# OrangeEarth15/3dgrut

Measured on AMD Instinct MI355X. Metric: train-step images/sec + render ms/frame, MipNeRF360 bicycle @1/2/4/8 GPU, higher is better.
Workload: dtype f32; 1 GPU; bicycle_like_6M_1237x822; num_gaussians=6000000, sh_degree=3, parallelism=per-view dp1, exchanged_records_last_step=0, loss=0.8*L1+0.2*(1-SSIM) (HIP fused SSIM), optimizer=HIP fused SH-gradient+Adam, all 59 params/Gaussian, trainer=native, optimizer_state=synthetic mid-training state: non-zero Adam moments on every row, storage_order=morton, optimizer_overlap=True, lazy_moment_decay=True, densification_statistics=False, warmup_extended_by=6

## Files before the change

3dgrut_amd/_capi.py:

```python
import ctypes as C
import os

HERE = os.path.dirname(os.path.abspath(__file__))
LIB_PATH = os.environ.get("GUT_HIP_LIB", os.path.join(HERE, "libgut_hip.so"))

GUT_ABI_VERSION = 6
GUT_NUM_KERNEL_TIMERS = 11
BWD_RAW_PARAMETER_GRADS = 1
BWD_COMPACT_RADIANCE_GRADS = 2
BWD_SKIP_EPILOGUE = 4
OPT_LAZY_TILE_ORDER = 1
ADAM_CLEAR_CONSUMED_GRADS = 1
GRADIENT_RECORD_FLOATS = 16
OPT_SORTED_REFERENCE_BACKWARD = 2
OPT_EARLY_EXTRA_PERCENT = 3
OPT_FORWARD_TILE_ORDER = 4
OPT_KERNEL_TIMING_SET = 5
OPT_DEBUG_REPLACE_SCRATCH = 100
KERNEL_TIMER_NAMES = ("project", "scan", "expand", "sort", "ranges", "render", "render_bwd", "project_bwd", "optimizer",
                      "optimizer_early", "optimizer_early_2")

SHUTTER_GLOBAL = 4
CAMERA_PINHOLE, CAMERA_FISHEYE = 0, 1

BUF = dict(tiles_count=0, tiles_offset=1, proj_pos=2, conic_opacity=3, extent=4, depth=5, feat=6,
           unsorted_keys=7, unsorted_ids=8, sorted_keys=9, sorted_ids=10, tile_ranges=11, grad_scratch=12,
           tile_traversed_fwd=13, tile_traversed_bwd=14, ordered_ids=15, packed_rows=16)


class GutCamera(C.Structure):
    _fields_ = [
        ("model", C.c_int32), ("shutter", C.c_int32),
        ("principal_point", C.c_float * 2), ("focal_length", C.c_float * 2),
        ("radial_coeffs", C.c_float * 6), ("tangential_coeffs", C.c_float * 2), ("thin_prism_coeffs", C.c_float * 4),
        ("max_angle", C.c_float), ("pose_start", C.c_float * 7), ("pose_end", C.c_float * 7),
        ("timestamp_start_us", C.c_int64), ("timestamp_end_us", C.c_int64),
    ]


class GutConfig(C.Structure):
    _fields_ = [
        ("abi_version", C.c_int32), ("enable_kernel_timings", C.c_int32), ("particle_radiance_sph_degree", C.c_int32),
        ("particle_kernel_degree", C.c_int32), ("k_buffer_size", C.c_int32), ("global_z_order", C.c_int32),
        ("n_rolling_shutter_iterations", C.c_int32), ("ut_require_all_sigma_points", C.c_int32),
        ("rect_bounding", C.c_int32), ("tight_opacity_bounding", C.c_int32), ("tile_based_culling", C.c_int32),
        ("enable_hitcounts", C.c_int32),
        ("particle_kernel_min_response", C.c_float), ("particle_kernel_min_alpha", C.c_float),
        ("particle_kernel_max_alpha", C.c_float), ("min_transmittance", C.c_float),
        ("ut_alpha", C.c_float), ("ut_beta", C.c_float), ("ut_kappa", C.c_float), ("ut_in_image_margin_factor", C.c_float),
    ]


class GutStats(C.Structure):
    _fields_ = [
        ("num_particles", C.c_uint64), ("num_visible", C.c_uint64), ("num_intersections", C.c_uint64),
        ("num_tiles", C.c_uint64), ("num_pixels", C.c_uint64), ("traversed_fwd", C.c_uint64),
        ("traversed_bwd", C.c_uint64), ("sort_end_bit", C.c_uint32), ("binning_overflows", C.c_uint32),
        ("side_stream_rows", C.c_uint64), ("side_stream_rows_first_launch", C.c_uint64),
    ]


class GutLazyMoments(C.Structure):
    _fields_ = [("d_wave_step", C.c_void_p), ("d_pow_beta1", C.c_void_p), ("d_pow_beta2", C.c_void_p), ("table_len", C.c_uint32),
                ("d_overrun", C.c_void_p)]


class GutRegularisation(C.Structure):
    _fields_ = [("density_coeff", C.c_float), ("scale_coeff", C.c_float), ("d_partials", C.c_void_p)]


EXPORTS = ("gut_default_config", "gut_create", "gut_destroy", "gut_trace", "gut_trace_bwd", "gut_collect_times",
           "gut_get_stats", "gut_debug_buffer", "gut_debug_copy", "gut_kernel_times", "gut_kernel_times_mean", "gut_last_error", "gut_abi_version",
           "gut_ssim_workspace_bytes", "gut_ssim_forward", "gut_ssim_backward",
           "gut_photometric_workspace_bytes", "gut_photometric_loss", "gut_optimize_after_bwd", "gut_set_option",
           "gut_trace_bwd_ex", "gut_optimize_rows_without_gradient", "gut_compact_gradient_rows", "gut_scatter_gradient_records",
           "gut_sh_adam_step_ex", "gut_mark_walked_waves", "gut_adam_unwalked_waves", "gut_activate_pack", "gut_adam_step", "gut_sh_adam_step", "gut_mcmc_relocation",
           "gut_optimize_finish_without_gradient", "gut_scatter_gradient_records_dev", "gut_adam_unwalked_waves_ex", "gut_sync_moments", "gut_trace_fields", "gut_trace_bwd_fields", "gut_selective_adam",
           "gut_trace_model_fields", "gut_trace_bwd_model_fields", "gut_position_gradient_statistics",
           "gut_set_position_gradient_statistics", "gut_mcmc_perturb", "gut_trace_raw_model_fields", "gut_set_regularisation",
           "gut_sh_adam_step_regularised", "gut_adam_unwalked_waves_regularised", "gut_sync_moments_ex", "gut_regularisation_gradient",
# ... 97 lines not shown
```

3dgrut_amd/csrc/gut_api.cpp:

```cpp
#include <hip/hip_runtime.h>

#include <cmath>
#include <cstdarg>
#include <cstdio>
#include <cstdlib>
#include <cstring>
#include <deque>
#include <mutex>
#include <new>
#include <string>

#include "gut_internal.h"

namespace {

thread_local std::string g_last_error;

int fail(const char* fmt, ...) {
    char buf[512];
    va_list ap;
    va_start(ap, fmt);
    vsnprintf(buf, sizeof(buf), fmt, ap);
    va_end(ap);
    g_last_error = buf;
// ... 1332 lines not shown
    case GUT_BUF_UNSORTED_KEYS:
    case GUT_BUF_UNSORTED_IDS:
    case GUT_BUF_SORTED_KEYS:
    case GUT_BUF_SORTED_IDS:
        if (h->lazy_order && !h->dbg_unsorted_valid && m) {
            DeviceGuard dev_guard;
            HIP_TRY(dev_guard.set(h->device));
            HIP_TRY(h->keys_unsorted.ensure(8 * m));
            HIP_TRY(h->ids_unsorted.ensure(4 * m));
            gut::launch_expand(h->fwd_stream, h->view, h->consts, (uint32_t)n, h->tiles_count.as<uint32_t>(), h->wave_sums.as<uint32_t>(),
                               h->block_prefix.as<uint32_t>(), h->scan_total.as<uint32_t>(), h->proj_pos.as<float>(),
                               h->conic_opacity.as<float>(), h->extent.as<float>(), h->depth.as<float>(),
                               h->keys_unsorted.as<uint64_t>(), h->ids_unsorted.as<uint32_t>(), (uint32_t)m);
            HIP_TRY(hipStreamSynchronize(h->fwd_stream));
            h->dbg_unsorted_valid = true;
        }
        if (which == GUT_BUF_UNSORTED_KEYS) { *d_ptr = h->keys_unsorted.p; *bytes = 8 * m; break; }
        if (which == GUT_BUF_UNSORTED_IDS) { *d_ptr = h->ids_unsorted.p; *bytes = 4 * m; break; }
        if (h->lazy_order) {
            if (!h->dbg_sorted_valid && m) {
                DeviceGuard dev_guard;
                HIP_TRY(dev_guard.set(h->device));
                HIP_TRY(h->dbg_keys_sorted.ensure(8 * m));
                HIP_TRY(h->dbg_ids_sorted.ensure(4 * m));
                DevBuf tmp;
                HIP_TRY(tmp.ensure(gut::sort_temp_bytes((uint32_t)m, h->end_bit)));
                hipError_t e = gut::run_sort(h->fwd_stream, tmp.p, tmp.cap, h->keys_unsorted.as<uint64_t>(),
                                             h->dbg_keys_sorted.as<uint64_t>(), h->ids_unsorted.as<uint32_t>(),
                                             h->dbg_ids_sorted.as<uint32_t>(), (uint32_t)m, h->end_bit);
                if (e == hipSuccess) e = hipStreamSynchronize(h->fwd_stream);
                tmp.release();
                HIP_TRY(e);
                h->dbg_sorted_valid = true;
            }
            if (which == GUT_BUF_SORTED_KEYS) { *d_ptr = h->dbg_keys_sorted.p; *bytes = 8 * m; }
            else { *d_ptr = h->dbg_ids_sorted.p; *bytes = 4 * m; }
        } else if (which == GUT_BUF_SORTED_KEYS) { *d_ptr = h->keys_sorted.p; *bytes = 8 * m; }
        else { *d_ptr = h->ids_sorted.p; *bytes = 4 * m; }
        break;
    case GUT_BUF_ORDERED_IDS:
        if (h->lazy_order && !h->dbg_ordered_valid && m) {
            DeviceGuard dev_guard;
            HIP_TRY(dev_guard.set(h->device));
            gut::launch_mask_unordered(h->fwd_stream, (uint32_t)h->tiles, h->ranges.as<uint32_t>(), h->tile_ordered.as<uint32_t>(),
                                       h->ids_ordered.as<uint32_t>());
            HIP_TRY(hipStreamSynchronize(h->fwd_stream));
            h->dbg_ordered_valid = true;
        }
        *d_ptr = h->lazy_order ? h->ids_ordered.p : h->ids_sorted.p; *bytes = 4 * m; break;
    case GUT_BUF_PACKED_ROWS:
        if (!h->packed_valid) return fail("gut_debug_buffer: the last forward was not a field-wise one (no packed rows)");
        *d_ptr = h->packed12.p; *bytes = 48 * n; break;
    case GUT_BUF_TILE_RANGES: *d_ptr = h->ranges.p; *bytes = 8 * t; break;
    case GUT_BUF_GRAD_SCRATCH:
        if (!h->have_backward) return fail("gut_debug_buffer: no backward yet");
        *d_ptr = h->grad16.p; *bytes = 64 * n; break;
    case GUT_BUF_TILE_TRAVERSED_FWD: *d_ptr = h->trav_fwd.p; *bytes = 4 * t; break;
    case GUT_BUF_TILE_TRAVERSED_BWD:
        if (!h->have_backward) return fail("gut_debug_buffer: no backward yet");
        *d_ptr = h->trav_bwd.p; *bytes = 4 * t; break;
    default: return fail("gut_debug_buffer: unknown buffer %d", which);
    }
    return 0;
}

int gut_debug_copy(gut_handle h, int32_t which, void* d_dst, size_t bytes) {
    void* src = nullptr;
    size_t have = 0;
    if (gut_debug_buffer(h, which, &src, &have)) return 1;
    if (bytes < have) return fail("gut_debug_copy: destination holds %zu bytes, buffer has %zu", bytes, have);
    if (have == 0) return 0;
    std::lock_guard<std::mutex> lock(h->mu);
    DeviceGuard dev_guard;
    HIP_TRY(dev_guard.set(h->device));
    HIP_TRY(hipMemcpyAsync(d_dst, src, have, hipMemcpyDeviceToDevice, h->fwd_stream));
    HIP_TRY(hipStreamSynchronize(h->fwd_stream));
    return 0;
}

}
```

3dgrut_amd/csrc/gut_project.hip:

```cpp
#include "gut_internal.h"

namespace gut {

__device__ __forceinline__ uint32_t f2u(float f) { return __float_as_uint(f); }
__device__ __forceinline__ float u2f(uint32_t u) { return __uint_as_float(u); }

__device__ float det_logf(float x) {
    uint32_t ix = f2u(x);
    int k = 0;
    if (ix >= 0x7f800000u) return x;
    if (ix < 0x00800000u) {
        if (ix == 0) return -__builtin_inff();
        x = x * 33554432.0f;
        ix = f2u(x);
        k -= 25;
    }
    k += (int)(ix >> 23) - 127;
    ix &= 0x007fffffu;
    const uint32_t i = (ix + (0x95f64u << 3)) & 0x800000u;
    x = u2f(ix | (i ^ 0x3f800000u));
    k += (int)(i >> 23);
    const float f = x - 1.0f;
    const float s = f / (2.0f + f);
    const float dk = (float)k;
// ... 222 lines not shown
        }
    }
}

__device__ __forceinline__ int clamp_tile(float v, int grid) {
    if (!(v > 0.0f)) return 0;
    if (v >= (float)grid) return grid;
    return (int)v;
}

struct TileBox {
    int x0, y0, x1, y1;
};

__device__ __forceinline__ TileBox tile_bbox(int gx, int gy, float px, float py, float ex, float ey) {
    TileBox b;
    b.x0 = clamp_tile(floorf((px - 0.5f - ex) / 16.0f), gx);
    b.y0 = clamp_tile(floorf((py - 0.5f - ey) / 16.0f), gy);
    b.x1 = clamp_tile(ceilf((px - 0.5f + ex) / 16.0f), gx);
    b.y1 = clamp_tile(ceilf((py - 0.5f + ey) / 16.0f), gy);
    return b;
}

__device__ __forceinline__ float saturate(float v) { return v > 0.0f ? (v < 1.0f ? v : 1.0f) : 0.0f; }

__device__ float tile_min_power(float tx, float ty, float c0, float c1, float c2, float mx, float my) {
    const float ts = 16.0f;
    const float tminx = ts * tx, tminy = ts * ty;
    const float tmaxx = ts + tminx, tmaxy = ts + tminy;
    const float offx = tminx - mx, offy = tminy - my;
    const float lax = offx > 0.0f ? 1.0f : 0.0f, lay = offy > 0.0f ? 1.0f : 0.0f;
    const float nrx = lax + (mx > tmaxx ? 1.0f : 0.0f);
    const float nry = lay + (my > tmaxy ? 1.0f : 0.0f);
    if ((nrx + nry) > 0.0f) {
        const float px = lax > 0.0f ? tminx : tmaxx;
        const float py = lay > 0.0f ? tminy : tmaxy;
        const float dxx = copysignf(ts, offx), dxy = copysignf(ts, offy);
        const float dfx = mx - px, dfy = my - py;
        const float rcx = 1.0f / (ts * ts * c0);
        const float rcy = 1.0f / (ts * ts * c2);
        const float tx_ = nry * saturate((dxx * c0 * dfx + dxx * c1 * dfy) * rcx);
        const float ty_ = nrx * saturate((dxy * c1 * dfx + dxy * c2 * dfy) * rcy);
        const float qx = mx - (px + tx_ * dxx);
        const float qy = my - (py + ty_ * dxy);
        return 0.5f * (c0 * qx * qx + c2 * qy * qy) + c1 * qx * qy;
    }
    return 0.0f;
}

constexpr int kSerialTiles = 12;
constexpr int kShRow = 49;

constexpr int kBinWindow = 1536;

struct TileWindow {
    int x0, y0, w, h;
};

__device__ TileWindow tile_window(const TileBox& bb, bool small, uint32_t* bins, int* red , uint32_t tid) {
    constexpr int kNone = 0x7fffffff;
    int a = small ? bb.x0 : kNone, b = small ? bb.y0 : kNone, c = small ? -bb.x1 : kNone, d = small ? -bb.y1 : kNone;
#pragma unroll
    for (int o = 32; o > 0; o >>= 1) {
        a = min(a, __shfl_xor(a, o));
        b = min(b, __shfl_xor(b, o));
        c = min(c, __shfl_xor(c, o));
        d = min(d, __shfl_xor(d, o));
    }
    if ((tid & 63u) == 0u) {
        red[4 * (tid >> 6) + 0] = a;
        red[4 * (tid >> 6) + 1] = b;
        red[4 * (tid >> 6) + 2] = c;
        red[4 * (tid >> 6) + 3] = d;
    }
    __syncthreads();
    a = __builtin_amdgcn_readfirstlane(min(min(red[0], red[4]), min(red[8], red[12])));
    b = __builtin_amdgcn_readfirstlane(min(min(red[1], red[5]), min(red[9], red[13])));
    c = __builtin_amdgcn_readfirstlane(min(min(red[2], red[6]), min(red[10], red[14])));
    d = __builtin_amdgcn_readfirstlane(min(min(red[3], red[7]), min(red[11], red[15])));
    TileWindow W = {0, 0, 0, 0};
    if (a != kNone && (-c - a) * (-d - b) <= kBinWindow) W = TileWindow{a, b, -c - a, -d - b};
    for (int k = (int)tid; k < W.w * W.h; k += kBlock) bins[k] = 0u;
    __syncthreads();
    return W;
}

__device__ __forceinline__ bool in_window(const TileWindow& W, int x, int y, uint32_t& bin) {
    const uint32_t bx = (uint32_t)(x - W.x0), by = (uint32_t)(y - W.y0);
    bin = by * (uint32_t)W.w + bx;
    return bx < (uint32_t)W.w && by < (uint32_t)W.h;
}

__device__ __forceinline__ uint32_t window_tile(const TileWindow& W, int grid_x, uint32_t bin) {
    const uint32_t by = bin / (uint32_t)W.w;
    return (uint32_t)(W.y0 + (int)by) * (uint32_t)grid_x + (uint32_t)W.x0 + (bin - by * (uint32_t)W.w);
}

__device__ __forceinline__ float bcast(float v, int src_lane) { return __shfl(v, src_lane); }
__device__ __forceinline__ int bcast(int v, int src_lane) { return __shfl(v, src_lane); }

template <int kVariant, bool kRolling, bool kSplitSH>
__global__ __launch_bounds__(kBlock, 5) void k_project_on_tiles(ViewParams v, RenderConsts c, uint32_t n, int sh_degree,
                                                            const float4* __restrict__ density12,
                                                            const float* __restrict__ sph48,
                                                            const float* __restrict__ sph_albedo,
                                                            uint32_t* __restrict__ tiles_count, float2* __restrict__ proj_pos,
                                                            float4* __restrict__ conic_opacity, float2* __restrict__ extent,
                                                            float* __restrict__ depth, float* __restrict__ feat,
                                                            float* __restrict__ visibility, uint32_t* __restrict__ wave_sums,
                                                            FrameClears clr) {
    __shared__ float sh_lds[(kBlock / 64) * 32 * kShRow];
    __shared__ uint32_t s_bins[kBinWindow];
    __shared__ int s_red[16];
    const uint32_t i = blockIdx.x * kBlock + threadIdx.x;
    const int lane = (int)(threadIdx.x & 63);
    const int wave = (int)(threadIdx.x >> 6);
    for (uint32_t t = i; t < clr.tiles; t += gridDim.x * kBlock) {
        clr.ranges[t] = make_uint2(0u, 0u);
        clr.trav_bwd[t] = 0u;
    }
    if (lane == 0 && clr.wave_walked) clr.wave_walked[blockIdx.x * (kBlock / 64) + (uint32_t)wave] = 0;
    if (i == 0 && clr.cam_pos) {
        clr.cam_pos[0] = v.s2w.t[0]; clr.cam_pos[1] = v.s2w.t[1]; clr.cam_pos[2] = v.s2w.t[2];
    }
    uint32_t cnt = 0;
    bool conic_ok = false, ok = false;
    float cx = 0.f, cy = 0.f, con0 = 0.f, con1 = 0.f, con2 = 0.f, con3 = 0.f, ex = 0.f, ey = 0.f, zkey = 0.f;
    float f0 = 0.f, f1 = 0.f, f2 = 0.f, max_power = 0.f, zcam = 0.f;
    float4 a = make_float4(0.f, 0.f, 0.f, 0.f);
    const uint32_t wave_first = blockIdx.x * kBlock + (uint32_t)wave * 64u;
    const uint32_t rows_here = wave_first < n ? min(64u, n - wave_first) : 0u;
    if (i < n) {
        a = density12[3 * (size_t)i + 0];
        const float4 b = density12[3 * (size_t)i + 1];
// ... 406 lines not shown
    if (serial) {
        for (int y = bb.y0; (y < bb.y1) && (off < max_off); ++y)
            for (int x = bb.x0; (x < bb.x1) && (off < max_off); ++x)
                if (tile_min_power((float)x, (float)y, con.x, con.y, con.z, p.x, p.y) < max_power) {
                    keys[off] = ((uint64_t)(uint32_t)(y * v.grid_x + x) << 32) | dkey;
                    ids[off] = i;
                    off++;
                }
    }
    unsigned long long todo = __ballot(active && area > kSerialTiles);
    while (todo) {
        const int j = __ffsll((long long)todo) - 1;
        todo &= todo - 1;
        const int jx0 = bcast(bb.x0, j), jy0 = bcast(bb.y0, j), jw = bcast(bb.x1 - bb.x0, j), jarea = bcast(area, j);
        const float j0 = bcast(con.x, j), j1 = bcast(con.y, j), j2 = bcast(con.z, j), jcx = bcast(p.x, j), jcy = bcast(p.y, j),
                    jmp = bcast(max_power, j);
        const uint32_t jdkey = (uint32_t)bcast((int)dkey, j), jmax = (uint32_t)bcast((int)max_off, j);
        const uint32_t jid = blockIdx.x * kBlock + (threadIdx.x & ~63u) + (uint32_t)j;
        uint32_t joff = (uint32_t)bcast((int)off, j);
        for (int base = 0; base < jarea; base += 64) {
            const int t = base + lane;
            bool pass = false;
            int tx = 0, ty = 0;
            if (t < jarea) {
                ty = t / jw;
                tx = t - ty * jw;
                pass = tile_min_power((float)(jx0 + tx), (float)(jy0 + ty), j0, j1, j2, jcx, jcy) < jmp;
            }
            const unsigned long long mask = __ballot(pass);
            const uint32_t my = joff + (uint32_t)__popcll(mask & ((1ull << lane) - 1ull));
            if (pass && my < jmax) {
                keys[my] = ((uint64_t)(uint32_t)((jy0 + ty) * v.grid_x + (jx0 + tx)) << 32) | jdkey;
                ids[my] = jid;
            }
            joff += (uint32_t)__popcll(mask);
        }
        if (lane == j) off = joff < jmax ? joff : jmax;
    }
    if (active)
        for (; off < max_off; ++off) {
            keys[off] = ((uint64_t)kInvalid << 32) | f2u(3.4028235e+38f);
            ids[off] = kInvalid;
        }
}

__global__ __launch_bounds__(kBlock) void k_expand_grouped(ViewParams v, RenderConsts c, uint32_t n,
                                                          const float2* __restrict__ proj_pos,
                                                          const float4* __restrict__ conic_opacity,
                                                          const float2* __restrict__ extent, const float* __restrict__ depth,
                                                          uint32_t tiles, const uint32_t* __restrict__ tile_start,
                                                          uint32_t* __restrict__ tile_cursor, uint2* __restrict__ ranges,
                                                          uint2* __restrict__ entries, uint32_t capacity) {
    __shared__ uint32_t s_bins[kBinWindow];
    __shared__ int s_red[16];
    const uint32_t i = blockIdx.x * kBlock + threadIdx.x;
    const int lane = (int)(threadIdx.x & 63);
    for (uint32_t t = i; t < tiles; t += gridDim.x * kBlock) {
        const uint32_t b = tile_start[t], e = tile_start[t + 1];
        ranges[t] = b == e ? make_uint2(0u, 0u) : make_uint2(min(b, capacity), min(e, capacity));
    }
    bool active = false;
    float2 e = make_float2(0.f, 0.f), p = make_float2(0.f, 0.f);
    float4 con = make_float4(0.f, 0.f, 0.f, 0.f);
    uint32_t dkey = 0;
    float max_power = 0.f;
    TileBox bb = {0, 0, 0, 0};
    int area = 0;
    if (i < n) {
        e = extent[i];
        active = !(e.x <= 1e-06f);
    }
    if (active) {
        dkey = f2u(depth[i]);
        p = proj_pos[i];
        bb = tile_bbox(v.grid_x, v.grid_y, p.x, p.y, e.x, e.y);
        area = (bb.x1 - bb.x0) * (bb.y1 - bb.y0);
        con = conic_opacity[i];
        if (c.tile_culling) max_power = det_logf(con.w / c.alpha_threshold);
    }
    const TileWindow W = tile_window(bb, active && area > 0 && area <= kSerialTiles, s_bins, s_red, threadIdx.x);
    auto enumerate = [&](auto emit) {
        if (!c.tile_culling) {
            if (active)
                for (int y = bb.y0; y < bb.y1; ++y)
                    for (int x = bb.x0; x < bb.x1; ++x) emit(x, y, i, dkey);
            return;
        }
        if (active && area <= kSerialTiles)
            for (int y = bb.y0; y < bb.y1; ++y)
                for (int x = bb.x0; x < bb.x1; ++x)
                    if (tile_min_power((float)x, (float)y, con.x, con.y, con.z, p.x, p.y) < max_power) emit(x, y, i, dkey);
        unsigned long long todo = __ballot(active && area > kSerialTiles);
        while (todo) {
            const int j = __ffsll((long long)todo) - 1;
            todo &= todo - 1;
            const int jx0 = bcast(bb.x0, j), jy0 = bcast(bb.y0, j), jw = bcast(bb.x1 - bb.x0, j), jarea = bcast(area, j);
            const float j0 = bcast(con.x, j), j1 = bcast(con.y, j), j2 = bcast(con.z, j), jcx = bcast(p.x, j), jcy = bcast(p.y, j),
                        jmp = bcast(max_power, j);
            const uint32_t jdkey = (uint32_t)bcast((int)dkey, j);
            const uint32_t jid = blockIdx.x * kBlock + (threadIdx.x & ~63u) + (uint32_t)j;
            for (int base = 0; base < jarea; base += 64) {
                const int t = base + lane;
                if (t < jarea) {
                    const int ty = t / jw;
                    const int tx = t - ty * jw;
                    if (tile_min_power((float)(jx0 + tx), (float)(jy0 + ty), j0, j1, j2, jcx, jcy) < jmp) emit(jx0 + tx, jy0 + ty, jid, jdkey);
                }
            }
        }
    };
    enumerate([&](int x, int y, uint32_t, uint32_t) {
        uint32_t bin;
        if (in_window(W, x, y, bin)) atomicAdd(&s_bins[bin], 1u);
    });
    __syncthreads();
    for (int k = (int)threadIdx.x; k < W.w * W.h; k += kBlock) {
        const uint32_t cnt = s_bins[k];
        if (cnt) s_bins[k] = atomicAdd(&tile_cursor[window_tile(W, v.grid_x, (uint32_t)k)], cnt);
    }
    __syncthreads();
    enumerate([&](int x, int y, uint32_t id, uint32_t dk) {
        uint32_t bin;
        const uint32_t slot = in_window(W, x, y, bin) ? atomicAdd(&s_bins[bin], 1u)
                                                      : atomicAdd(&tile_cursor[(uint32_t)y * (uint32_t)v.grid_x + (uint32_t)x], 1u);
        if (slot < capacity) entries[slot] = make_uint2(dk, id);
    });
}

__global__ __launch_bounds__(kBlock) void k_pad_keys(const uint32_t* __restrict__ count, uint32_t sort_n, uint64_t* __restrict__ keys,
                                                    uint32_t* __restrict__ ids) {
    const uint32_t m = *count;
    for (uint32_t k = m + blockIdx.x * kBlock + threadIdx.x; k < sort_n; k += gridDim.x * kBlock) {
        keys[k] = ((uint64_t)kInvalid << 32) | f2u(3.4028235e+38f);
        ids[k] = kInvalid;
    }
}

__global__ __launch_bounds__(kBlock) void k_mask_unordered(uint32_t tiles, const uint2* __restrict__ ranges,
                                                          const uint32_t* __restrict__ tile_ordered, uint32_t* __restrict__ ordered_ids) {
    const uint32_t t = blockIdx.x;
    if (t >= tiles) return;
    const uint2 r = ranges[t];
    for (uint32_t k = r.x + min(r.y - r.x, tile_ordered[t]) + threadIdx.x; k < r.y; k += kBlock) ordered_ids[k] = kInvalid;
}

void launch_mask_unordered(hipStream_t s, uint32_t tiles, const uint32_t* ranges, const uint32_t* tile_ordered, uint32_t* ordered_ids) {
    if (tiles == 0) return;
    hipLaunchKernelGGL(k_mask_unordered, dim3(tiles), dim3(kBlock), 0, s, tiles, reinterpret_cast<const uint2*>(ranges), tile_ordered,
                       ordered_ids);
}

void launch_pad_keys(hipStream_t s, const uint32_t* count, uint32_t sort_n, uint64_t* keys, uint32_t* ids) {
    if (sort_n == 0) return;
    hipLaunchKernelGGL(k_pad_keys, dim3(64), dim3(kBlock), 0, s, count, sort_n, keys, ids);
}

__global__ __launch_bounds__(kBlock) void k_tile_ranges(uint32_t m, const uint64_t* __restrict__ sorted_keys,
                                                       uint2* __restrict__ ranges) {
    const uint32_t k = blockIdx.x * kBlock + threadIdx.x;
    if (k >= m) return;
    const uint32_t tile = (uint32_t)(sorted_keys[k] >> 32);
    const bool valid = tile != kInvalid;
    if (k == 0) {
        if (valid) ranges[tile].x = 0;
    } else {
        const uint32_t prev = (uint32_t)(sorted_keys[k - 1] >> 32);
        if (prev != tile) {
            if (prev != kInvalid) ranges[prev].y = k;
            if (valid) ranges[tile].x = k;
        }
    }
    if (valid && (k == m - 1)) ranges[tile].y = m;
}

template <bool kRawGrads, bool kSplitSH>
__global__ __launch_bounds__(kBlock) void k_project_backward(ViewParams v, uint32_t n, int sh_degree,
                                                            const float4* __restrict__ density12,
// ... 261 lines not shown
```

3dgrut_amd/tracer.py:

```python
import ctypes as C
import enum
import math
import os

import numpy as np
import torch

from . import _capi
from .cameras import ShutterType as DatasetShutterType
from .pose import SensorPose3D, sensor_pose_from_c2w


class ShutterType(enum.IntEnum):
    ROLLING_TOP_TO_BOTTOM = 0
    ROLLING_LEFT_TO_RIGHT = 1
    ROLLING_BOTTOM_TO_TOP = 2
    ROLLING_RIGHT_TO_LEFT = 3
    GLOBAL = 4


SHUTTER_TYPE_MAP = {d: ShutterType[d.name] for d in DatasetShutterType}


def plugin_shutter_type(value):
# ... 400 lines not shown
        with torch.cuda.device(act12.device):
            rc = self._lib.gut_compact_gradient_rows(self._handle, C.c_void_p(stream), act12.data_ptr(), records.data_ptr(),
                                                     int(records.shape[0]), count.data_ptr())
        _capi.check(rc, "compact_gradient_rows")

    def collect_times(self):
        f, b = C.c_float(-1.0), C.c_float(-1.0)
        _capi.check(self._lib.gut_collect_times(self._handle, C.byref(f), C.byref(b)), "collect_times")
        if f.value >= 0:
            self._timings["forward_render"] = f.value
        if b.value >= 0:
            self._timings["backward_render"] = b.value
        return dict(self._timings)

    def set_lazy_tile_order(self, on=True):
        _capi.check(self._lib.gut_set_option(self._handle, _capi.OPT_LAZY_TILE_ORDER, 1 if on else 0), "set_option")

    def set_early_extra_percent(self, percent):
        _capi.check(self._lib.gut_set_option(self._handle, _capi.OPT_EARLY_EXTRA_PERCENT, int(percent)), "set_option")

    def set_forward_tile_order(self, mode):
        _capi.check(self._lib.gut_set_option(self._handle, _capi.OPT_FORWARD_TILE_ORDER, int(mode)), "set_option")

    def set_kernel_timing_set(self, which):
        _capi.check(self._lib.gut_set_option(self._handle, _capi.OPT_KERNEL_TIMING_SET, int(which)), "set_option")

    def debug_replace_scratch(self, index):
        _capi.check(self._lib.gut_set_option(self._handle, _capi.OPT_DEBUG_REPLACE_SCRATCH, int(index)), "set_option")

    def set_sorted_reference_backward(self, on=True):
        _capi.check(self._lib.gut_set_option(self._handle, _capi.OPT_SORTED_REFERENCE_BACKWARD, 1 if on else 0), "set_option")

    def stats(self):
        s = _capi.GutStats()
        _capi.check(self._lib.gut_get_stats(self._handle, C.byref(s)), "stats")
        return {k: int(getattr(s, k)) for k, _ in s._fields_ if k != "reserved"}

    def kernel_times(self):
        arr = (C.c_float * _capi.GUT_NUM_KERNEL_TIMERS)()
        _capi.check(self._lib.gut_kernel_times(self._handle, arr), "kernel_times")
        return dict(zip(_capi.KERNEL_TIMER_NAMES, [float(v) for v in arr]))

    def kernel_times_mean(self):
        arr = (C.c_float * _capi.GUT_NUM_KERNEL_TIMERS)()
        cnt = C.c_int32(0)
        _capi.check(self._lib.gut_kernel_times_mean(self._handle, arr, C.byref(cnt)), "kernel_times_mean")
        return dict(zip(_capi.KERNEL_TIMER_NAMES, [float(v) for v in arr])), int(cnt.value)

    def debug_buffer(self, name, device=None):
        ptr, nbytes = C.c_void_p(), C.c_size_t()
        _capi.check(self._lib.gut_debug_buffer(self._handle, _capi.BUF[name], C.byref(ptr), C.byref(nbytes)), "debug_buffer")
        dt = {"tiles_count": torch.int32, "tiles_offset": torch.int32, "unsorted_ids": torch.int32,
              "sorted_ids": torch.int32, "ordered_ids": torch.int32, "tile_ranges": torch.int32, "tile_traversed_fwd": torch.int32,
              "tile_traversed_bwd": torch.int32, "unsorted_keys": torch.int64,
              "sorted_keys": torch.int64}.get(name, torch.float32)
        n = nbytes.value // (8 if dt == torch.int64 else 4)
        dev = torch.device("cuda", self.device_index) if device is None else device
        out = torch.empty(n, dtype=dt, device=dev)
        if n:
            _capi.check(self._lib.gut_debug_copy(self._handle, _capi.BUF[name], C.c_void_p(out.data_ptr()),
                                                 C.c_size_t(nbytes.value)), "debug_copy")
        return out


class Tracer:
    class _Autograd(torch.autograd.Function):
        @staticmethod
        def forward(ctx, tracer_wrapper, frame_id, n_active_features, ray_ori, ray_dir, mog_pos, mog_rot, mog_scl,
                    mog_dns, mog_sph, sensor_params, sensor_poses, mog_sph_specular=None, raw_parameters=False):
            ctx.frame_id = frame_id
            ctx.n_active_features = n_active_features
            ctx.sensor_params = sensor_params
            ctx.sensor_poses = sensor_poses
            ctx.tracer_wrapper = tracer_wrapper
            ctx.set_materialize_grads(False)
            ctx.model_fields = mog_sph_specular is not None
            if ctx.model_fields:
                trace = tracer_wrapper.trace_raw_model_fields if raw_parameters else tracer_wrapper.trace_model_fields
                rgba, dist, hits, vis = trace(
                    frame_id, n_active_features, mog_pos, mog_dns, mog_rot, mog_scl, mog_sph.contiguous(), mog_sph_specular.contiguous(),
                    ray_ori.contiguous(), ray_dir.contiguous(), sensor_params, sensor_poses.timestamps_us[0],
                    sensor_poses.timestamps_us[1], sensor_poses.T_world_sensors[0], sensor_poses.T_world_sensors[1])
                ctx.fields = True
                ctx.num_particles = int(mog_pos.shape[0])
                ctx.save_for_backward(ray_ori, ray_dir, rgba, dist)
                ctx.mark_non_differentiable(hits, vis)
                return rgba, dist, hits, vis
            particle_radiance = mog_sph.contiguous()
            ctx.fields = hasattr(tracer_wrapper, "trace_fields")
            if ctx.fields:
                rgba, dist, hits, vis = tracer_wrapper.trace_fields(
                    frame_id, n_active_features, mog_pos, mog_dns, mog_rot, mog_scl, particle_radiance, ray_ori.contiguous(),
                    ray_dir.contiguous(), sensor_params, sensor_poses.timestamps_us[0], sensor_poses.timestamps_us[1],
                    sensor_poses.T_world_sensors[0], sensor_poses.T_world_sensors[1])
                ctx.num_particles = int(mog_pos.shape[0])
                ctx.save_for_backward(ray_ori, ray_dir, rgba, dist, particle_radiance)
                ctx.mark_non_differentiable(hits, vis)
                return rgba, dist, hits, vis
            particle_density = torch.cat([mog_pos, mog_dns, mog_rot, mog_scl, torch.zeros_like(mog_dns)], dim=1).contiguous()
            ray_time = None
            rgba, dist, hits, vis = tracer_wrapper.trace(
                frame_id, n_active_features, particle_density, particle_radiance, ray_ori.contiguous(),
                ray_dir.contiguous(), ray_time, sensor_params, sensor_poses.timestamps_us[0], sensor_poses.timestamps_us[1],
                sensor_poses.T_world_sensors[0], sensor_poses.T_world_sensors[1])
            ctx.save_for_backward(ray_ori, ray_dir, rgba, dist, particle_density, particle_radiance)
            ctx.mark_non_differentiable(hits, vis)
            return rgba, dist, hits, vis
# ... 114 lines not shown
```

include/gut_hip.h:

```cpp
#ifndef GUT_HIP_H
#define GUT_HIP_H

#include <stddef.h>
#include <stdint.h>

#ifdef __cplusplus
extern "C" {
#endif

#define GUT_ABI_VERSION 6

typedef struct gut_context* gut_handle;

enum { GUT_SHUTTER_ROLLING_TOP_TO_BOTTOM = 0, GUT_SHUTTER_ROLLING_LEFT_TO_RIGHT = 1,
       GUT_SHUTTER_ROLLING_BOTTOM_TO_TOP = 2, GUT_SHUTTER_ROLLING_RIGHT_TO_LEFT = 3, GUT_SHUTTER_GLOBAL = 4 };
enum { GUT_CAMERA_OPENCV_PINHOLE = 0, GUT_CAMERA_OPENCV_FISHEYE = 1 };

typedef struct GutCamera {
    int32_t model;
    int32_t shutter;
    float principal_point[2];
    float focal_length[2];
    float radial_coeffs[6];
    float tangential_coeffs[2];
// ... 5 lines not shown
    int64_t timestamp_end_us;
} GutCamera;

typedef struct GutConfig {
    int32_t abi_version;
    int32_t enable_kernel_timings;
    int32_t particle_radiance_sph_degree;
    int32_t particle_kernel_degree;
    int32_t k_buffer_size;
    int32_t global_z_order;
    int32_t n_rolling_shutter_iterations;
    int32_t ut_require_all_sigma_points;
    int32_t rect_bounding, tight_opacity_bounding, tile_based_culling;
    int32_t enable_hitcounts;
    float particle_kernel_min_response;
    float particle_kernel_min_alpha;
    float particle_kernel_max_alpha;
    float min_transmittance;
    float ut_alpha, ut_beta, ut_kappa;
    float ut_in_image_margin_factor;
} GutConfig;

typedef struct GutStats {
    uint64_t num_particles;
    uint64_t num_visible;
    uint64_t num_intersections;
    uint64_t num_tiles;
    uint64_t num_pixels;
    uint64_t traversed_fwd;
    uint64_t traversed_bwd;
    uint32_t sort_end_bit;
    uint32_t binning_overflows;
    uint64_t side_stream_rows;
    uint64_t side_stream_rows_first_launch;
} GutStats;

enum {
    GUT_BUF_TILES_COUNT = 0,
    GUT_BUF_TILES_OFFSET = 1,
    GUT_BUF_PROJ_POSITION = 2,
    GUT_BUF_CONIC_OPACITY = 3,
    GUT_BUF_PROJ_EXTENT = 4,
    GUT_BUF_GLOBAL_DEPTH = 5,
    GUT_BUF_FEATURES = 6,
    GUT_BUF_UNSORTED_KEYS = 7,
    GUT_BUF_UNSORTED_IDS = 8,
    GUT_BUF_SORTED_KEYS = 9,
    GUT_BUF_SORTED_IDS = 10,
    GUT_BUF_TILE_RANGES = 11,
    GUT_BUF_GRAD_SCRATCH = 12,
    GUT_BUF_TILE_TRAVERSED_FWD = 13,
    GUT_BUF_TILE_TRAVERSED_BWD = 14,
    GUT_BUF_ORDERED_IDS = 15,
    GUT_BUF_PACKED_ROWS = 16
};

void gut_default_config(GutConfig* cfg);

int gut_create(const GutConfig* cfg, int device_index, gut_handle* out);
void gut_destroy(gut_handle h);

int gut_trace(gut_handle h, void* stream, uint32_t frame_number, int32_t num_active_features ,
              uint32_t num_particles, const float* d_particle_density, const float* d_particle_radiance,
              int32_t width, int32_t height, const float* d_ray_origin, const float* d_ray_direction,
              const GutCamera* camera,
              float* d_ray_radiance_density, float* d_ray_hit_distance, float* d_ray_hit_count,
              float* d_particle_visibility);

int gut_trace_bwd(gut_handle h, void* stream, uint32_t frame_number, int32_t num_active_features,
                  uint32_t num_particles, const float* d_particle_density, const float* d_particle_radiance,
                  int32_t width, int32_t height, const float* d_ray_origin, const float* d_ray_direction,
                  const GutCamera* camera,
                  const float* d_ray_radiance_density, const float* d_ray_radiance_density_grad,
                  const float* d_ray_hit_distance, const float* d_ray_hit_distance_grad,
                  float* d_particle_density_grad, float* d_particle_radiance_grad);

#define GUT_BWD_RAW_PARAMETER_GRADS 1u
#define GUT_BWD_COMPACT_RADIANCE_GRADS 2u
#define GUT_BWD_SKIP_EPILOGUE 4u
int gut_trace_bwd_ex(gut_handle h, void* stream, uint32_t frame_number, int32_t num_active_features,
                     uint32_t num_particles, const float* d_particle_density, const float* d_particle_radiance,
                     int32_t width, int32_t height, const float* d_ray_origin, const float* d_ray_direction,
                     const GutCamera* camera,
                     const float* d_ray_radiance_density, const float* d_ray_radiance_density_grad,
                     const float* d_ray_hit_distance, const float* d_ray_hit_distance_grad,
                     float* d_particle_density_grad, float* d_particle_radiance_grad, uint32_t flags);

int gut_trace_fields(gut_handle h, void* stream, uint32_t frame_number, int32_t num_active_features, uint32_t num_particles,
                     const float* d_positions, const float* d_density, const float* d_rotation, const float* d_scale,
                     const float* d_particle_radiance, int32_t width, int32_t height, const float* d_ray_origin,
                     const float* d_ray_direction, const GutCamera* camera, float* d_ray_radiance_density,
                     float* d_ray_hit_distance, float* d_ray_hit_count, float* d_particle_visibility);
int gut_trace_bwd_fields(gut_handle h, void* stream, uint32_t frame_number, int32_t num_active_features, uint32_t num_particles,
                         const float* d_particle_radiance, int32_t width, int32_t height, const float* d_ray_origin,
                         const float* d_ray_direction, const GutCamera* camera, const float* d_ray_radiance_density,
                         const float* d_ray_radiance_density_grad, const float* d_ray_hit_distance,
                         const float* d_ray_hit_distance_grad, float* d_positions_grad, float* d_density_grad, float* d_rotation_grad,
                         float* d_scale_grad, float* d_particle_radiance_grad);

int gut_trace_model_fields(gut_handle h, void* stream, uint32_t frame_number, int32_t num_active_features, uint32_t num_particles,
                           const float* d_positions, const float* d_density, const float* d_rotation, const float* d_scale,
                           const float* d_features_albedo, const float* d_features_specular, int32_t width, int32_t height,
                           const float* d_ray_origin, const float* d_ray_direction, const GutCamera* camera,
                           float* d_ray_radiance_density, float* d_ray_hit_distance, float* d_ray_hit_count,
                           float* d_particle_visibility);
int gut_trace_raw_model_fields(gut_handle h, void* stream, uint32_t frame_number, int32_t num_active_features, uint32_t num_particles,
                               const float* d_positions, const float* d_density_logit, const float* d_rotation_raw, const float* d_log_scale,
// ... 147 lines not shown
```

Measured before the change: 468.8 images/s.

## Bin small-box tile entries once with cached ranks and widen shared bin window

The tile-binning kernel now culls each small Gaussian's tiles once, records the pass mask and its shared-memory rank, and reuses them in the emit pass instead of re-running culling. The shared bin window can also cover boxes of up to 256 tiles, with separate 16-bit counts for small and large contributors and a second shared array of cursors for large boxes. The goal is fewer repeated tile_min_power evaluations and fewer global tile_cursor atomics. In exchange it uses more shared memory, packs counts into 16 bits, and packs ranks into 8 bits, which could overflow if many entries fall in one bin.

```diff
diff --git a/3dgrut_amd/_capi.py b/3dgrut_amd/_capi.py
--- a/3dgrut_amd/_capi.py
+++ b/3dgrut_amd/_capi.py
@@ -25,7 +25,7 @@
 
 BUF = dict(tiles_count=0, tiles_offset=1, proj_pos=2, conic_opacity=3, extent=4, depth=5, feat=6,
            unsorted_keys=7, unsorted_ids=8, sorted_keys=9, sorted_ids=10, tile_ranges=11, grad_scratch=12,
-           tile_traversed_fwd=13, tile_traversed_bwd=14, ordered_ids=15, packed_rows=16)
+           tile_traversed_fwd=13, tile_traversed_bwd=14, ordered_ids=15, packed_rows=16, grouped_entries=17)
 
 
 class GutCamera(C.Structure):
diff --git a/3dgrut_amd/csrc/gut_api.cpp b/3dgrut_amd/csrc/gut_api.cpp
--- a/3dgrut_amd/csrc/gut_api.cpp
+++ b/3dgrut_amd/csrc/gut_api.cpp
@@ -1408,6 +1408,9 @@
         if (!h->packed_valid) return fail("gut_debug_buffer: the last forward was not a field-wise one (no packed rows)");
         *d_ptr = h->packed12.p; *bytes = 48 * n; break;
     case GUT_BUF_TILE_RANGES: *d_ptr = h->ranges.p; *bytes = 8 * t; break;
+    case GUT_BUF_GROUPED_ENTRIES:
+        if (!h->lazy_order && m) return fail("gut_debug_buffer: the last forward sorted its list (no grouped entries)");
+        *d_ptr = h->keys_sorted.p; *bytes = 8 * m; break;
     case GUT_BUF_GRAD_SCRATCH:
         if (!h->have_backward) return fail("gut_debug_buffer: no backward yet");
         *d_ptr = h->grad16.p; *bytes = 64 * n; break;
diff --git a/3dgrut_amd/csrc/gut_project.hip b/3dgrut_amd/csrc/gut_project.hip
--- a/3dgrut_amd/csrc/gut_project.hip
+++ b/3dgrut_amd/csrc/gut_project.hip
@@ -298,14 +298,16 @@
 constexpr int kShRow = 49;
 
 constexpr int kBinWindow = 1536;
+constexpr int kWideTiles = 256;
 
 struct TileWindow {
     int x0, y0, w, h;
 };
 
-__device__ TileWindow tile_window(const TileBox& bb, bool small, uint32_t* bins, int* red , uint32_t tid) {
-    constexpr int kNone = 0x7fffffff;
-    int a = small ? bb.x0 : kNone, b = small ? bb.y0 : kNone, c = small ? -bb.x1 : kNone, d = small ? -bb.y1 : kNone;
+constexpr int kNoBox = 0x7fffffff;
+
+__device__ __forceinline__ void wave_box_union(const TileBox& bb, bool take, int* red, uint32_t tid) {
+    int a = take ? bb.x0 : kNoBox, b = take ? bb.y0 : kNoBox, c = take ? -bb.x1 : kNoBox, d = take ? -bb.y1 : kNoBox;
 #pragma unroll
     for (int o = 32; o > 0; o >>= 1) {
         a = min(a, __shfl_xor(a, o));
@@ -314,18 +316,38 @@
         d = min(d, __shfl_xor(d, o));
     }
     if ((tid & 63u) == 0u) {
-        red[4 * (tid >> 6) + 0] = a;
-        red[4 * (tid >> 6) + 1] = b;
-        red[4 * (tid >> 6) + 2] = c;
-        red[4 * (tid >> 6) + 3] = d;
-    }
+        red[0] = a;
+        red[1] = b;
+        red[2] = c;
+        red[3] = d;
+    }
+}
+
+__device__ __forceinline__ TileWindow block_box_union(const int* red) {
+    const int a = __builtin_amdgcn_readfirstlane(min(min(red[0], red[4]), min(red[8], red[12])));
+    const int b = __builtin_amdgcn_readfirstlane(min(min(red[1], red[5]), min(red[9], red[13])));
+    const int c = __builtin_amdgcn_readfirstlane(min(min(red[2], red[6]), min(red[10], red[14])));
+    const int d = __builtin_amdgcn_readfirstlane(min(min(red[3], red[7]), min(red[11], red[15])));
+    TileWindow W = {0, 0, 0, 0};
+    if (a != kNoBox && (-c - a) * (-d - b) <= kBinWindow) W = TileWindow{a, b, -c - a, -d - b};
+    return W;
+}
+
+__device__ TileWindow tile_window(const TileBox& bb, bool small, uint32_t* bins, int* red , uint32_t tid) {
+    wave_box_union(bb, small, red + 4 * (tid >> 6), tid);
     __syncthreads();
-    a = __builtin_amdgcn_readfirstlane(min(min(red[0], red[4]), min(red[8], red[12])));
-    b = __builtin_amdgcn_readfirstlane(min(min(red[1], red[5]), min(red[9], red[13])));
-    c = __builtin_amdgcn_readfirstlane(min(min(red[2], red[6]), min(red[10], red[14])));
-    d = __builtin_amdgcn_readfirstlane(min(min(red[3], red[7]), min(red[11], red[15])));
-    TileWindow W = {0, 0, 0, 0};
-    if (a != kNone && (-c - a) * (-d - b) <= kBinWindow) W = TileWindow{a, b, -c - a, -d - b};
+    const TileWindow W = block_box_union(red);
+    for (int k = (int)tid; k < W.w * W.h; k += kBlock) bins[k] = 0u;
+    __syncthreads();
+    return W;
+}
+
+__device__ TileWindow tile_window_wide(const TileBox& bb, bool small, bool wide, uint32_t* bins, int* red , uint32_t tid) {
+    wave_box_union(bb, small, red + 4 * (tid >> 6), tid);
+    wave_box_union(bb, wide, red + 16 + 4 * (tid >> 6), tid);
+    __syncthreads();
+    TileWindow W = block_box_union(red + 16);
+    if (W.w == 0) W = block_box_union(red);
     for (int k = (int)tid; k < W.w * W.h; k += kBlock) bins[k] = 0u;
     __syncthreads();
     return W;
@@ -838,7 +860,8 @@
                                                           uint32_t* __restrict__ tile_cursor, uint2* __restrict__ ranges,
                                                           uint2* __restrict__ entries, uint32_t capacity) {
     __shared__ uint32_t s_bins[kBinWindow];
-    __shared__ int s_red[16];
+    __shared__ uint32_t s_large[kBinWindow];
+    __shared__ int s_red[32];
     const uint32_t i = blockIdx.x * kBlock + threadIdx.x;
     const int lane = (int)(threadIdx.x & 63);
     for (uint32_t t = i; t < tiles; t += gridDim.x * kBlock) {
@@ -864,18 +887,29 @@
         con = conic_opacity[i];
         if (c.tile_culling) max_power = det_logf(con.w / c.alpha_threshold);
     }
-    const TileWindow W = tile_window(bb, active && area > 0 && area <= kSerialTiles, s_bins, s_red, threadIdx.x);
-    auto enumerate = [&](auto emit) {
-        if (!c.tile_culling) {
-            if (active)
-                for (int y = bb.y0; y < bb.y1; ++y)
-                    for (int x = bb.x0; x < bb.x1; ++x) emit(x, y, i, dkey);
-            return;
-        }
-        if (active && area <= kSerialTiles)
-            for (int y = bb.y0; y < bb.y1; ++y)
-                for (int x = bb.x0; x < bb.x1; ++x)
-                    if (tile_min_power((float)x, (float)y, con.x, con.y, con.z, p.x, p.y) < max_power) emit(x, y, i, dkey);
+    const bool small = active && area > 0 && area <= kSerialTiles;
+    const TileWindow W = tile_window_wide(bb, small, active && area > 0 && area <= kWideTiles, s_bins, s_red, threadIdx.x);
+    const bool cull = c.tile_culling != 0;
+    const uint32_t grid_x = (uint32_t)v.grid_x;
+    uint32_t pass = 0u, rank[3] = {0u, 0u, 0u};
+    if (small) {
+        int x = bb.x0, y = bb.y0;
+#pragma unroll
+        for (int t = 0; t < kSerialTiles; ++t) {
+            if (t < area) {
+                if (!cull || tile_min_power((float)x, (float)y, con.x, con.y, con.z, p.x, p.y) < max_power) {
+                    pass |= 1u << t;
+                    uint32_t bin;
+                    if (in_window(W, x, y, bin)) rank[t >> 2] |= (atomicAdd(&s_bins[bin], 1u) & 0xffffu) << (8 * (t & 3));
+                }
+                if (++x == bb.x1) {
+                    x = bb.x0;
+                    ++y;
+                }
+            }
+        }
+    }
+    auto for_large_boxes = [&](auto emit) {
         unsigned long long todo = __ballot(active && area > kSerialTiles);
         while (todo) {
             const int j = __ffsll((long long)todo) - 1;
@@ -890,25 +924,48 @@
                 if (t < jarea) {
                     const int ty = t / jw;
                     const int tx = t - ty * jw;
-                    if (tile_min_power((float)(jx0 + tx), (float)(jy0 + ty), j0, j1, j2, jcx, jcy) < jmp) emit(jx0 + tx, jy0 + ty, jid, jdkey);
+                    if (!cull || tile_min_power((float)(jx0 + tx), (float)(jy0 + ty), j0, j1, j2, jcx, jcy) < jmp)
+                        emit(jx0 + tx, jy0 + ty, jid, jdkey);
                 }
             }
         }
     };
-    enumerate([&](int x, int y, uint32_t, uint32_t) {
+    for_large_boxes([&](int x, int y, uint32_t, uint32_t) {
         uint32_t bin;
-        if (in_window(W, x, y, bin)) atomicAdd(&s_bins[bin], 1u);
+        if (in_window(W, x, y, bin)) atomicAdd(&s_bins[bin], 0x10000u);
     });
     __syncthreads();
     for (int k = (int)threadIdx.x; k < W.w * W.h; k += kBlock) {
         const uint32_t cnt = s_bins[k];
-        if (cnt) s_bins[k] = atomicAdd(&tile_cursor[window_tile(W, v.grid_x, (uint32_t)k)], cnt);
+        if (cnt) {
+            const uint32_t first = atomicAdd(&tile_cursor[window_tile(W, v.grid_x, (uint32_t)k)], (cnt & 0xffffu) + (cnt >> 16));
+            s_large[k] = first;
+            s_bins[k] = first + (cnt >> 16);
+        }
     }
     __syncthreads();
-    enumerate([&](int x, int y, uint32_t id, uint32_t dk) {
+    if (pass) {
+        int x = bb.x0, y = bb.y0;
+#pragma unroll
+        for (int t = 0; t < kSerialTiles; ++t) {
+            if (t < area) {
+                if ((pass >> t) & 1u) {
+                    uint32_t bin;
+                    const uint32_t slot = in_window(W, x, y, bin) ? s_bins[bin] + ((rank[t >> 2] >> (8 * (t & 3))) & 0xffu)
+                                                                  : atomicAdd(&tile_cursor[(uint32_t)y * grid_x + (uint32_t)x], 1u);
+                    if (slot < capacity) entries[slot] = make_uint2(dkey, i);
+                }
+                if (++x == bb.x1) {
+                    x = bb.x0;
+                    ++y;
+                }
+            }
+        }
+    }
+    for_large_boxes([&](int x, int y, uint32_t id, uint32_t dk) {
         uint32_t bin;
-        const uint32_t slot = in_window(W, x, y, bin) ? atomicAdd(&s_bins[bin], 1u)
-                                                      : atomicAdd(&tile_cursor[(uint32_t)y * (uint32_t)v.grid_x + (uint32_t)x], 1u);
+        const uint32_t slot = in_window(W, x, y, bin) ? atomicAdd(&s_large[bin], 1u)
+                                                      : atomicAdd(&tile_cursor[(uint32_t)y * grid_x + (uint32_t)x], 1u);
         if (slot < capacity) entries[slot] = make_uint2(dk, id);
     });
 }
diff --git a/3dgrut_amd/tracer.py b/3dgrut_amd/tracer.py
--- a/3dgrut_amd/tracer.py
+++ b/3dgrut_amd/tracer.py
@@ -476,7 +476,7 @@
         _capi.check(self._lib.gut_debug_buffer(self._handle, _capi.BUF[name], C.byref(ptr), C.byref(nbytes)), "debug_buffer")
         dt = {"tiles_count": torch.int32, "tiles_offset": torch.int32, "unsorted_ids": torch.int32,
               "sorted_ids": torch.int32, "ordered_ids": torch.int32, "tile_ranges": torch.int32, "tile_traversed_fwd": torch.int32,
-              "tile_traversed_bwd": torch.int32, "unsorted_keys": torch.int64,
+              "tile_traversed_bwd": torch.int32, "grouped_entries": torch.int32, "unsorted_keys": torch.int64,
               "sorted_keys": torch.int64}.get(name, torch.float32)
         n = nbytes.value // (8 if dt == torch.int64 else 4)
         dev = torch.device("cuda", self.device_index) if device is None else device
diff --git a/include/gut_hip.h b/include/gut_hip.h
--- a/include/gut_hip.h
+++ b/include/gut_hip.h
@@ -81,7 +81,8 @@
     GUT_BUF_TILE_TRAVERSED_FWD = 13,
     GUT_BUF_TILE_TRAVERSED_BWD = 14,
     GUT_BUF_ORDERED_IDS = 15,
-    GUT_BUF_PACKED_ROWS = 16
+    GUT_BUF_PACKED_ROWS = 16,
+    GUT_BUF_GROUPED_ENTRIES = 17
 };
 
 void gut_default_config(GutConfig* cfg);
```

Result: faster. 475.5 images/s, median of 5 (+1.4%).
